# cocowy1/PPMStereo

Measured on AMD Instinct MI355X. Metric: disparity-px/s, higher is better.
Workload: dtype bf16; 1 GPU; BASELINE config 2: T=5 clip at 320x512, iters=10, hot path only (3-scale cascade from encoder outputs: corr pyramid build + lookup, QAM pick, pick-and-play memory attention, ConvGRU3D update, heads, convex upsample, test_mode=True as PPMStereo.forward_batch_test calls it: predictions[-1] is the output, so the mask head, the convex upsampling and the full-resolution resize run only where their resu; T=5, H=320, W=512, iters=10, parallelism=replicas x1

## Files before the change

### ppmstereo_amd/csrc/pwchain.hip

```cpp
#include "common.h"

namespace {

constexpr int TP = 128;
constexpr int ROWB = 64;
constexpr int ACT_PLANE = TP * ROWB;
constexpr int ACT_BUF = 4 * ACT_PLANE;
constexpr int W_BLK = 2 * 2 * 64 * 64;

__device__ __forceinline__ int swzp(int row, int chunk) { return row * 64 + ((chunk ^ ((row >> 2) & 3)) << 4); }

struct Layer {
    const void* w;
    const float* bias;
    const float* post_s;
    const float* post_t;
    int M;
    int n_valid;
    int resid;
};

struct ChainParams {
    ppms_sp in, out;
    Layer layer[3];
    int nlayers;
    int64_t P;
};

__global__ __launch_bounds__(256) void pwchain_kernel(const ChainParams* __restrict__ cp) {
    extern __shared__ __attribute__((aligned(16))) char smem[];
    const ChainParams& c = *cp;
    char* bufX = smem;
    char* bufA = smem + ACT_BUF;
    char* wsm = smem + 2 * ACT_BUF;
    const int tid = threadIdx.x, lane = tid & 63, wave = tid >> 6;
    const int r = lane & 31, h = lane >> 5;
    const int64_t p0 = (int64_t)blockIdx.x * TP;

    for (int q = tid; q < TP * 8; q += 256) {
        const int px = q >> 3, ch = q & 7;
        const int64_t pix = p0 + px;
        u32x4 vh = {0, 0, 0, 0}, vl = {0, 0, 0, 0};
        if (pix < c.P) {
            vh = gload16((const bf16_t*)c.in.hi + pix * c.in.ld + ch * 8);
            vl = gload16((const bf16_t*)c.in.lo + pix * c.in.ld + ch * 8);
        }
        const int off = (ch >> 2) * 2 * ACT_PLANE + swzp(px, ch & 3);
        *(u32x4*)(bufX + off) = vh;
        *(u32x4*)(bufX + ACT_PLANE + off) = vl;
    }
    u32x4 wreg[4];
    auto load_w = [&](int l, int mblk) __attribute__((always_inline)) {
        const Layer& Lw = c.layer[l];
        const int mbs = Lw.M / 64;
#pragma unroll
        for (int i = 0; i < 4; ++i) {
            const int q = tid + i * 256;
            const int ks = q >> 9, rem = q & 511;
            wreg[i] = gload16((const char*)Lw.w + ((int64_t)(ks * mbs + mblk) * 512 + rem) * 16);
        }
    };
    load_w(0, 0);
    const char* src = bufX;
    for (int l = 0; l < c.nlayers; ++l) {
        const Layer& L = c.layer[l];
        const bool last = (l == c.nlayers - 1);
        char* dst = (src == bufX) ? bufA : bufX;
        const int mblocks = L.M / 64;
        for (int mblk = 0; mblk < mblocks; ++mblk) {
            __syncthreads();
#pragma unroll
            for (int i = 0; i < 4; ++i) *(u32x4*)(wsm + (tid + i * 256) * 16) = wreg[i];
            if (mblk + 1 < mblocks)
                load_w(l, mblk + 1);
            else if (l + 1 < c.nlayers)
                load_w(l + 1, 0);
            __syncthreads();
            f32x16 acc[2];
            acc[0] = (f32x16){0};
            acc[1] = (f32x16){0};
#pragma unroll
            for (int ks = 0; ks < 2; ++ks) {
#pragma unroll
                for (int k16 = 0; k16 < 2; ++k16) {
                    const int boff = ks * 2 * ACT_PLANE + swzp(wave * 32 + r, 2 * k16 + h);
                    const bf16x8 bh = *(const bf16x8*)(src + boff);
                    const bf16x8 bl = *(const bf16x8*)(src + ACT_PLANE + boff);
#pragma unroll
                    for (int mb = 0; mb < 2; ++mb) {
                        const int aoff = ks * 8192 + swzp(mb * 32 + r, 2 * k16 + h);
                        const bf16x8 ah = *(const bf16x8*)(wsm + aoff);
                        const bf16x8 al = *(const bf16x8*)(wsm + 4096 + aoff);
                        acc[mb] = __builtin_amdgcn_mfma_f32_32x32x16_bf16(al, bh, acc[mb], 0, 0, 0);
                        acc[mb] = __builtin_amdgcn_mfma_f32_32x32x16_bf16(ah, bl, acc[mb], 0, 0, 0);
                        acc[mb] = __builtin_amdgcn_mfma_f32_32x32x16_bf16(ah, bh, acc[mb], 0, 0, 0);
                    }
                }
            }
            const int px = wave * 32 + r;
            const int64_t pix = p0 + px;
#pragma unroll
            for (int mb = 0; mb < 2; ++mb)
#pragma unroll
                for (int g = 0; g < 4; ++g) {
                    const int cl = mb * 32 + 8 * g + 4 * h;
                    const int cg = mblk * 64 + cl;
                    const f32x4 b4 = gld<f32x4>(L.bias + cg);
                    float y[4];
#pragma unroll
                    for (int j = 0; j < 4; ++j) y[j] = acc[mb][4 * g + j] + b4[j];
                    if (L.resid) {
                        const int xo = (cl >> 5) * 2 * ACT_PLANE + swzp(px, (cl & 31) >> 3) + (cl & 7) * 2;
                        const bf16x4 xh = *(const bf16x4*)(bufX + xo), xl = *(const bf16x4*)(bufX + ACT_PLANE + xo);
#pragma unroll
                        for (int j = 0; j < 4; ++j) y[j] += join_bf16(xh[j], xl[j]);
                    }
#pragma unroll
                    for (int j = 0; j < 4; ++j) y[j] = gelu_erf(y[j]);
                    if (L.post_s != nullptr) {
                        const f32x4 s4 = gld<f32x4>(L.post_s + cg), t4 = gld<f32x4>(L.post_t + cg);
#pragma unroll
                        for (int j = 0; j < 4; ++j) y[j] = gelu_erf(y[j] + (y[j] * s4[j] + t4[j]));
                    }
                    bf16x4 oh, ol;
#pragma unroll
                    for (int j = 0; j < 4; ++j) {
                        bf16_t hh = (bf16_t)0.0f, ll = (bf16_t)0.0f;
                        if (cg + j < L.n_valid) split_bf16(y[j], hh, ll);
                        oh[j] = hh;
                        ol[j] = ll;
                    }
                    {
                        const int xo = (cl >> 5) * 2 * ACT_PLANE + swzp(px, (cl & 31) >> 3) + (cl & 7) * 2;
                        *(bf16x4*)(dst + xo) = oh;
                        *(bf16x4*)(dst + ACT_PLANE + xo) = ol;
                    }
                }
            if (last) {
                __syncthreads();
                for (int qd = tid; qd < TP * 16; qd += 256) {
                    const int opx = qd >> 4, plane = (qd >> 3) & 1, ch = qd & 7;
                    const int64_t opix = p0 + opx;
                    const int ocg = mblk * 64 + ch * 8;
                    if (opix < c.P && ocg < L.n_valid) {
                        const u32x4 v = *(const u32x4*)(dst + (ch >> 2) * 2 * ACT_PLANE + plane * ACT_PLANE + swzp(opx, ch & 3));
                        bf16_t* op = (bf16_t*)(plane ? c.out.lo : c.out.hi) + opix * c.out.ld + ocg;
                        if (ocg + 8 <= L.n_valid) {
                            gstore16(op, v);
                        } else {
                            const bf16_t* e = (const bf16_t*)&v;
                            for (int j = 0; j < 8; ++j)
                                if (ocg + j < L.n_valid) gst<bf16_t>(op + j, e[j]);
                        }
                    }
                }
            }
        }
        src = dst;
    }
}

constexpr int TP32 = 32;
constexpr int ACT32_PLANE = TP32 * ROWB;
constexpr int ACT32_BUF = 4 * ACT32_PLANE;
constexpr int W32_MAX = 4 * W_BLK;

__global__ __launch_bounds__(256) void pwchain32_kernel(const ChainParams* __restrict__ cp) {
    extern __shared__ __attribute__((aligned(16))) char smem[];
    const ChainParams& c = *cp;
    char* bufX = smem;
    char* bufA = smem + ACT32_BUF;
    char* wsm = smem + 2 * ACT32_BUF;
    const int tid = threadIdx.x, lane = tid & 63, wave = tid >> 6;
    const int r = lane & 31, h = lane >> 5;
    const int64_t p0 = (int64_t)blockIdx.x * TP32;
    {
        const int px = tid >> 3, ch = tid & 7;
        const int64_t pix = p0 + px;
        u32x4 vh = {0, 0, 0, 0}, vl = {0, 0, 0, 0};
        if (pix < c.P) {
            vh = gload16((const bf16_t*)c.in.hi + pix * c.in.ld + ch * 8);
            vl = gload16((const bf16_t*)c.in.lo + pix * c.in.ld + ch * 8);
        }
        const int off = (ch >> 2) * 2 * ACT32_PLANE + swzp(px, ch & 3);
        *(u32x4*)(bufX + off) = vh;
        *(u32x4*)(bufX + ACT32_PLANE + off) = vl;
    }
    u32x4 wreg[16];
    auto load_w = [&](int l) __attribute__((always_inline)) {
        const Layer& Lw = c.layer[l];
        const int mbs = Lw.M / 64;
#pragma unroll
        for (int mblk = 0; mblk < 4; ++mblk)
            if (mblk < mbs) {
#pragma unroll
                for (int i = 0; i < 4; ++i) {
                    const int q = tid + i * 256;
                    const int ks = q >> 9, rem = q & 511;
                    wreg[mblk * 4 + i] = gload16((const char*)Lw.w + ((int64_t)(ks * mbs + mblk) * 512 + rem) * 16);
                }
            }
    };
    load_w(0);
    const char* src = bufX;
    for (int l = 0; l < c.nlayers; ++l) {
        const Layer& L = c.layer[l];
        const bool last = (l == c.nlayers - 1);
        char* dst = (src == bufX) ? bufA : bufX;
        const int mbs = L.M / 64, nrb = L.M / 32;
        __syncthreads();
#pragma unroll
        for (int mblk = 0; mblk < 4; ++mblk)
            if (mblk < mbs) {
#pragma unroll
                for (int i = 0; i < 4; ++i) *(u32x4*)(wsm + mblk * W_BLK + (tid + i * 256) * 16) = wreg[mblk * 4 + i];
            }
        if (l + 1 < c.nlayers) load_w(l + 1);
        __syncthreads();
        bf16x4 keep_h[2][4], keep_l[2][4];
#pragma unroll
        for (int it = 0; it < 2; ++it) {
            const int rb = wave + 4 * it;
            if (rb >= nrb) continue;
            const int mblk = rb >> 1, mb = rb & 1;
            f32x16 acc = (f32x16){0};
#pragma unroll
            for (int ks = 0; ks < 2; ++ks)
#pragma unroll
                for (int k16 = 0; k16 < 2; ++k16) {
                    const int boff = ks * 2 * ACT32_PLANE + swzp(r, 2 * k16 + h);
                    const bf16x8 bh = *(const bf16x8*)(src + boff), bl = *(const bf16x8*)(src + ACT32_PLANE + boff);
                    const int aoff = mblk * W_BLK + ks * 8192 + swzp(mb * 32 + r, 2 * k16 + h);
                    const bf16x8 ah = *(const bf16x8*)(wsm + aoff), al = *(const bf16x8*)(wsm + 4096 + aoff);
                    acc = __builtin_amdgcn_mfma_f32_32x32x16_bf16(al, bh, acc, 0, 0, 0);
                    acc = __builtin_amdgcn_mfma_f32_32x32x16_bf16(ah, bl, acc, 0, 0, 0);
                    acc = __builtin_amdgcn_mfma_f32_32x32x16_bf16(ah, bh, acc, 0, 0, 0);
                }
#pragma unroll
            for (int g = 0; g < 4; ++g) {
                const int cl = mb * 32 + 8 * g + 4 * h;
                const int cg = mblk * 64 + cl;
                const f32x4 b4 = gld<f32x4>(L.bias + cg);
                float y[4];
#pragma unroll
                for (int j = 0; j < 4; ++j) y[j] = acc[4 * g + j] + b4[j];
                const int xo = (cl >> 5) * 2 * ACT32_PLANE + swzp(r, (cl & 31) >> 3) + (cl & 7) * 2;
                if (L.resid) {
                    const bf16x4 xh = *(const bf16x4*)(bufX + xo), xl = *(const bf16x4*)(bufX + ACT32_PLANE + xo);
#pragma unroll
                    for (int j = 0; j < 4; ++j) y[j] += join_bf16(xh[j], xl[j]);
                }
#pragma unroll
                for (int j = 0; j < 4; ++j) y[j] = gelu_erf(y[j]);
                if (L.post_s != nullptr) {
                    const f32x4 s4 = gld<f32x4>(L.post_s + cg), t4 = gld<f32x4>(L.post_t + cg);
#pragma unroll
                    for (int j = 0; j < 4; ++j) y[j] = gelu_erf(y[j] + (y[j] * s4[j] + t4[j]));
                }
                bf16x4 oh, ol;
#pragma unroll
                for (int j = 0; j < 4; ++j) {
                    bf16_t hh = (bf16_t)0.0f, ll = (bf16_t)0.0f;
                    if (cg + j < L.n_valid) split_bf16(y[j], hh, ll);
                    oh[j] = hh;
                    ol[j] = ll;
                }
                if (last) {
                    keep_h[it][g] = oh;
                    keep_l[it][g] = ol;
                } else {
                    *(bf16x4*)(dst + xo) = oh;
                    *(bf16x4*)(dst + ACT32_PLANE + xo) = ol;
                }
            }
        }
        if (last) {
            __syncthreads();
            const int rowb = L.M * 2 + 16;
#pragma unroll
            for (int it = 0; it < 2; ++it) {
                const int rb = wave + 4 * it;
                if (rb >= nrb) continue;
#pragma unroll
                for (int g = 0; g < 4; ++g) {
                    const int cg = rb * 32 + 8 * g + 4 * h;
                    *(bf16x4*)(wsm + r * rowb + cg * 2) = keep_h[it][g];
                    *(bf16x4*)(wsm + TP32 * rowb + r * rowb + cg * 2) = keep_l[it][g];
                }
            }
            __syncthreads();
            const int cpr = L.M / 8;
            for (int qd = tid; qd < TP32 * 2 * cpr; qd += 256) {
                const int plane = qd / (TP32 * cpr), rem = qd - plane * TP32 * cpr;
                const int opx = rem / cpr, ch = rem - opx * cpr;
                const int64_t opix = p0 + opx;
                const int ocg = ch * 8;
                if (opix < c.P && ocg < L.n_valid) {
                    const u32x4 v = *(const u32x4*)(wsm + plane * TP32 * rowb + opx * rowb + ocg * 2);
                    bf16_t* op = (bf16_t*)(plane ? c.out.lo : c.out.hi) + opix * c.out.ld + ocg;
                    if (ocg + 8 <= L.n_valid) {
                        gstore16(op, v);
                    } else {
                        const bf16_t* e = (const bf16_t*)&v;
                        for (int j = 0; j < 8; ++j)
                            if (ocg + j < L.n_valid) gst<bf16_t>(op + j, e[j]);
                    }
                }
            }
        }
        src = dst;
    }
}

}

static int pwchain_launch(const void* dev_params, int64_t pixels, void* stream) {
    constexpr size_t lds = 2 * ACT_BUF + W_BLK;
    constexpr size_t lds32 = 2 * ACT32_BUF + W32_MAX;
    static ppms_device_once once;
    once.run([] {
        (void)hipFuncSetAttribute((const void*)pwchain_kernel, hipFuncAttributeMaxDynamicSharedMemorySize, (int)(2 * ACT_BUF + W_BLK));
        (void)hipFuncSetAttribute((const void*)pwchain32_kernel, hipFuncAttributeMaxDynamicSharedMemorySize, (int)(2 * ACT32_BUF + W32_MAX));
    });
    if (pixels <= 16384) {
        hipLaunchKernelGGL(pwchain32_kernel, dim3(ceil_div(pixels, TP32)), dim3(256), lds32, (hipStream_t)stream, (const ChainParams*)dev_params);
        return ppms_check_launch("pwchain");
    }
    hipLaunchKernelGGL(pwchain_kernel, dim3(ceil_div(pixels, TP)), dim3(256), lds, (hipStream_t)stream, (const ChainParams*)dev_params);
    return ppms_check_launch("pwchain");
}

extern "C" int ppms_pwchain(const void* dev_params, int64_t pixels, void* stream) {
    PPMS_REQUIRE(dev_params != nullptr && pixels > 0, "pwchain: bad arguments");
    return pwchain_launch(dev_params, pixels, stream);
}

extern "C" int ppms_pwchain_param_bytes(void) { return (int)sizeof(ChainParams); }
```

### ppmstereo_amd/csrc/small_ops.hip

```cpp
#include "common.h"

static thread_local char g_err[512] = "";
void ppms_set_error(const char* fmt, ...) {
    va_list ap;
    va_start(ap, fmt);
    vsnprintf(g_err, sizeof(g_err), fmt, ap);
    va_end(ap);
}
int ppms_check_launch(const char* what) {
    hipError_t e = hipGetLastError();
    if (e != hipSuccess) {
        ppms_set_error("%s: HIP launch failed: %s", what, hipGetErrorString(e));
        return PPMS_ELAUNCH;
    }
    return PPMS_OK;
}
extern "C" const char* ppms_last_error(void) { return g_err; }
extern "C" int ppms_version(void) { return PPMS_ABI_VERSION; }
extern "C" int ppms_struct_sizes(int* sp, int* epilogue, int* conv) {
    if (sp) *sp = (int)sizeof(ppms_sp);
    if (epilogue) *epilogue = (int)sizeof(ppms_epilogue);
    if (conv) *conv = (int)sizeof(ppms_conv);
    return PPMS_OK;
}
extern "C" int ppms_device_info(char* name, int name_cap, int* cu_count, int* clock_mhz) {
    int dev = 0;
    if (hipGetDevice(&dev) != hipSuccess) {
        ppms_set_error("no HIP device");
        return PPMS_ENODEV;
    }
    hipDeviceProp_t prop;
    if (hipGetDeviceProperties(&prop, dev) != hipSuccess) {
        ppms_set_error("hipGetDeviceProperties failed");
        return PPMS_ENODEV;
    }
    if (name && name_cap > 0) snprintf(name, name_cap, "%s", prop.gcnArchName);
    if (cu_count) *cu_count = prop.multiProcessorCount;
    if (clock_mhz) *clock_mhz = prop.clockRate / 1000;
    return PPMS_OK;
}

constexpr int DW_PX = 2;
template <int K>
__global__ __launch_bounds__(256) void dwconv_gelu_kernel(ppms_sp x, ppms_sp y, const float* __restrict__ w, const float* __restrict__ b,
                                                          int H, int W, int64_t rows, int groups) {
    __shared__ __attribute__((aligned(16))) float wl[K * K * 64];
    const int C = groups * 8;
    for (int i = threadIdx.x; i < K * K * C; i += 256) {
        const int c = i % C, tap = i / C;
        wl[tap * C + c] = w[c * K * K + tap];
    }
    __syncthreads();
    const int rpr = (W + DW_PX - 1) / DW_PX;
    const int64_t idx = (int64_t)blockIdx.x * 256 + threadIdx.x;
    if (idx >= rows * rpr * groups) return;
    const int c0 = (int)(idx % groups) * 8;
    const int64_t run = idx / groups;
    const int px0 = (int)(run % rpr) * DW_PX;
    const int64_t row = run / rpr;
    const int py = (int)(row % H);
    const int64_t pix0 = row * W + px0;
    const bf16_t* xh = (const bf16_t*)x.hi + c0;
    const bf16_t* xl = (const bf16_t*)x.lo + c0;
    float acc[DW_PX][8], x0[DW_PX][8];
    {
        const f32x4 b0 = *(const f32x4*)(b + c0), b1 = *(const f32x4*)(b + c0 + 4);
#pragma unroll
        for (int p = 0; p < DW_PX; ++p)
#pragma unroll
            for (int j = 0; j < 8; ++j) {
                acc[p][j] = j < 4 ? b0[j & 3] : b1[j & 3];
                x0[p][j] = 0.0f;
            }
    }
    constexpr int R = K / 2, NW = DW_PX + K - 1;
#pragma unroll
    for (int ky = 0; ky < K; ++ky) {
        const int yy = py + ky - R;
        if ((unsigned)yy >= (unsigned)H) continue;
        float win[NW][8];
#pragma unroll
        for (int i = 0; i < NW; ++i) {
            const int xx = px0 - R + i;
            bf16x8 h8 = {0, 0, 0, 0, 0, 0, 0, 0}, l8 = {0, 0, 0, 0, 0, 0, 0, 0};
            if ((unsigned)xx < (unsigned)W) {
                const int64_t q = pix0 + (int64_t)(ky - R) * W + (i - R);
                h8 = *(const bf16x8*)(xh + q * x.ld);
                l8 = *(const bf16x8*)(xl + q * x.ld);
            }
#pragma unroll
            for (int j = 0; j < 8; ++j) win[i][j] = join_bf16(h8[j], l8[j]);
        }
        if (ky == R) {
#pragma unroll
            for (int p = 0; p < DW_PX; ++p)
#pragma unroll
                for (int j = 0; j < 8; ++j) x0[p][j] = win[p + R][j];
        }
#pragma unroll
        for (int kx = 0; kx < K; ++kx) {
            const f32x4 w0 = *(const f32x4*)(wl + (ky * K + kx) * C + c0), w1 = *(const f32x4*)(wl + (ky * K + kx) * C + c0 + 4);
#pragma unroll
            for (int p = 0; p < DW_PX; ++p)
#pragma unroll
                for (int j = 0; j < 8; ++j) acc[p][j] += (j < 4 ? w0[j & 3] : w1[j & 3]) * win[p + kx][j];
        }
    }
#pragma unroll
    for (int p = 0; p < DW_PX; ++p) {
        if (px0 + p >= W) break;
        bf16x8 oh, ol;
#pragma unroll
        for (int j = 0; j < 8; ++j) {
            bf16_t hi, lo;
            split_bf16(gelu_erf(x0[p][j] + acc[p][j]), hi, lo);
            oh[j] = hi;
            ol[j] = lo;
        }
        *(bf16x8*)((bf16_t*)y.hi + (pix0 + p) * y.ld + c0) = oh;
        *(bf16x8*)((bf16_t*)y.lo + (pix0 + p) * y.ld + c0) = ol;
    }
}

extern "C" int ppms_dwconv_gelu(ppms_sp x, ppms_sp y, const float* w, const float* b, int k, int BT, int H, int W, void* stream) {
    PPMS_REQUIRE(k == 1 || k == 7, "dwconv_gelu: k=%d (only 1 and 7)", k);
    PPMS_REQUIRE(x.hi && x.lo && y.hi && y.lo && x.c == y.c && x.c > 0 && x.c <= 64 && x.c % 8 == 0 && x.ld % 8 == 0 && y.ld % 8 == 0,
                 "dwconv_gelu: views must have c <= 64 and c, ld multiples of 8");
    const int64_t rows = (int64_t)BT * H;
    const int groups = x.c / 8;
    const dim3 grid(ceil_div(rows * ((W + DW_PX - 1) / DW_PX) * groups, 256));
    if (k == 1)
        hipLaunchKernelGGL(dwconv_gelu_kernel<1>, grid, dim3(256), 0, (hipStream_t)stream, x, y, w, b, H, W, rows, groups);
    else
        hipLaunchKernelGGL(dwconv_gelu_kernel<7>, grid, dim3(256), 0, (hipStream_t)stream, x, y, w, b, H, W, rows, groups);
    return ppms_check_launch("dwconv_gelu");
}

__global__ __launch_bounds__(256) void flow_patch7_kernel(const float* __restrict__ flow, ppms_sp patch, int H, int W, int64_t P) {
    const int64_t idx = (int64_t)blockIdx.x * 256 + threadIdx.x;
    if (idx >= P * 128) return;
    const int k = (int)(idx & 127);
    const int64_t pix = idx >> 7;
    float v = 0.0f;
    if (k < 98) {
        const int tap = k >> 1, c = k & 1;
        const int ky = tap / 7, kx = tap - ky * 7;
        const int px = (int)(pix % W), py = (int)((pix / W) % H);
        const int xx = px + kx - 3, yy = py + ky - 3;
        if ((unsigned)xx < (unsigned)W && (unsigned)yy < (unsigned)H) v = flow[(pix + (int64_t)(ky - 3) * W + (kx - 3)) * 2 + c];
    }
    bf16_t hi, lo;
    split_bf16(v, hi, lo);
    ((bf16_t*)patch.hi)[pix * patch.ld + k] = hi;
    ((bf16_t*)patch.lo)[pix * patch.ld + k] = lo;
}

extern "C" int ppms_flow_patch7(const float* flow_nhwc, ppms_sp patch, int BT, int H, int W, void* stream) {
    PPMS_REQUIRE(flow_nhwc && patch.hi && patch.lo && patch.ld >= 128, "flow_patch7: bad arguments");
    const int64_t P = (int64_t)BT * H * W;
    hipLaunchKernelGGL(flow_patch7_kernel, dim3(ceil_div(P * 128, 256)), dim3(256), 0, (hipStream_t)stream, flow_nhwc, patch, H, W, P);
    return ppms_check_launch("flow_patch7");
}

__global__ __launch_bounds__(256) void unc_tail_kernel(ppms_sp x, const float* __restrict__ w, float bias, float* __restrict__ unc,
                                                       float* __restrict__ partial, int HW, int nblk) {
    __shared__ float red[16];
    const int frame = blockIdx.y, blk = blockIdx.x;
    const int sub = threadIdx.x & 15, grp = threadIdx.x >> 4;
    float wv[8];
#pragma unroll
    for (int j = 0; j < 8; ++j) wv[j] = w[sub * 8 + j];
    bf16x8 h8[16], l8[16];
#pragma unroll
    for (int it = 0; it < 16; ++it) {
        const int pin = blk * 256 + it * 16 + grp;
        const int64_t pix = (int64_t)frame * HW + (pin < HW ? pin : HW - 1);
        h8[it] = gld<bf16x8>((const bf16_t*)x.hi + pix * x.ld + sub * 8);
        l8[it] = gld<bf16x8>((const bf16_t*)x.lo + pix * x.ld + sub * 8);
    }
    float local = 0.0f;
#pragma unroll
    for (int it = 0; it < 16; ++it) {
        const int pin = blk * 256 + it * 16 + grp;
        float s = 0.0f;
#pragma unroll
        for (int j = 0; j < 8; ++j) s += wv[j] * join_bf16(h8[it][j], l8[it][j]);
        s += __shfl_xor(s, 1);
        s += __shfl_xor(s, 2);
        s += __shfl_xor(s, 4);
        s += __shfl_xor(s, 8);
        if (pin < HW && sub == 0) {
            const float u = sigmoid_f(s + bias);
            unc[(int64_t)frame * HW + pin] = u;
            local += u;
        }
    }
    if (sub == 0) red[grp] = local;
    __syncthreads();
    if (threadIdx.x == 0) {
        float t = 0.0f;
        for (int i = 0; i < 16; ++i) t += red[i];
        partial[frame * nblk + blk] = t;
    }
}

extern "C" int ppms_unc_tail(ppms_sp x, const float* w, float bias, float* unc, float* partial, int BT, int HW, void* stream) {
    PPMS_REQUIRE(x.hi && x.lo && x.c == 128 && x.ld % 8 == 0, "unc_tail: expects a 128-channel SP view");
    const int nblk = ceil_div(HW, 256);
    hipLaunchKernelGGL(unc_tail_kernel, dim3(nblk, BT), dim3(256), 0, (hipStream_t)stream, x, w, bias, unc, partial, HW, nblk);
    return ppms_check_launch("unc_tail");
}

enum { CV_F32 = 0, CV_SP = 1 };
template <int DST_KIND>
__global__ __launch_bounds__(256) void nchw_to_cl_kernel(const float* __restrict__ src, float* __restrict__ dst_f32, int dst_ld,
                                                         ppms_sp dst_sp, int C, int HW) {
    __shared__ float tile[32][33];
    const int frame = blockIdx.z;
    const int c0 = blockIdx.y * 32, p0 = blockIdx.x * 32;
    const int tx = threadIdx.x & 31, ty = threadIdx.x >> 5;
    for (int i = ty; i < 32; i += 8) {
        const int c = c0 + i, p = p0 + tx;
        tile[i][tx] = (c < C && p < HW) ? src[((int64_t)frame * C + c) * HW + p] : 0.0f;
    }
    __syncthreads();
    for (int i = ty; i < 32; i += 8) {
        const int p = p0 + i, c = c0 + tx;
        if (p < HW && c < C) {
            const float v = tile[tx][i];
            const int64_t pix = (int64_t)frame * HW + p;
            if (DST_KIND == CV_F32) {
                dst_f32[pix * dst_ld + c] = v;
            } else {
                bf16_t hi, lo;
                split_bf16(v, hi, lo);
                ((bf16_t*)dst_sp.hi)[pix * dst_sp.ld + c] = hi;
                ((bf16_t*)dst_sp.lo)[pix * dst_sp.ld + c] = lo;
            }
        }
    }
}
template <int SRC_KIND>
__global__ __launch_bounds__(256) void cl_to_nchw_kernel(const float* __restrict__ src_f32, int src_ld, ppms_sp src_sp,
                                                         float* __restrict__ dst, int C, int HW) {
    __shared__ float tile[32][33];
    const int frame = blockIdx.z;
    const int c0 = blockIdx.y * 32, p0 = blockIdx.x * 32;
    const int tx = threadIdx.x & 31, ty = threadIdx.x >> 5;
    for (int i = ty; i < 32; i += 8) {
        const int p = p0 + i, c = c0 + tx;
        float v = 0.0f;
        if (p < HW && c < C) {
            const int64_t pix = (int64_t)frame * HW + p;
            if (SRC_KIND == CV_F32)
                v = src_f32[pix * src_ld + c];
            else
                v = join_bf16(((const bf16_t*)src_sp.hi)[pix * src_sp.ld + c], ((const bf16_t*)src_sp.lo)[pix * src_sp.ld + c]);
        }
        tile[i][tx] = v;
    }
    __syncthreads();
    for (int i = ty; i < 32; i += 8) {
        const int c = c0 + i, p = p0 + tx;
        if (c < C && p < HW) dst[((int64_t)frame * C + c) * HW + p] = tile[tx][i];
    }
}

extern "C" int ppms_nchw_to_sp(const float* src, ppms_sp dst, int BT, int C, int HW, void* stream) {
    PPMS_REQUIRE(src && dst.hi && dst.lo && dst.ld >= C, "nchw_to_sp: bad arguments");
    hipLaunchKernelGGL(nchw_to_cl_kernel<CV_SP>, dim3(ceil_div(HW, 32), ceil_div(C, 32), BT), dim3(256), 0, (hipStream_t)stream, src,
                       (float*)nullptr, 0, dst, C, HW);
    return ppms_check_launch("nchw_to_sp");
}
extern "C" int ppms_nchw_to_nhwc(const float* src, float* dst, int dst_ld, int BT, int C, int HW, void* stream) {
    PPMS_REQUIRE(src && dst && dst_ld >= C, "nchw_to_nhwc: bad arguments");
    ppms_sp none = {nullptr, nullptr, 0, 0};
    hipLaunchKernelGGL(nchw_to_cl_kernel<CV_F32>, dim3(ceil_div(HW, 32), ceil_div(C, 32), BT), dim3(256), 0, (hipStream_t)stream, src, dst,
                       dst_ld, none, C, HW);
    return ppms_check_launch("nchw_to_nhwc");
}
extern "C" int ppms_sp_to_nchw(ppms_sp src, float* dst, int BT, int C, int HW, void* stream) {
    PPMS_REQUIRE(dst && src.hi && src.lo && src.ld >= C, "sp_to_nchw: bad arguments");
    hipLaunchKernelGGL(cl_to_nchw_kernel<CV_SP>, dim3(ceil_div(HW, 32), ceil_div(C, 32), BT), dim3(256), 0, (hipStream_t)stream,
                       (const float*)nullptr, 0, src, dst, C, HW);
    return ppms_check_launch("sp_to_nchw");
}
extern "C" int ppms_nhwc_to_nchw(const float* src, int src_ld, float* dst, int BT, int C, int HW, void* stream) {
    PPMS_REQUIRE(src && dst && src_ld >= C, "nhwc_to_nchw: bad arguments");
    ppms_sp none = {nullptr, nullptr, 0, 0};
    hipLaunchKernelGGL(cl_to_nchw_kernel<CV_F32>, dim3(ceil_div(HW, 32), ceil_div(C, 32), BT), dim3(256), 0, (hipStream_t)stream, src,
                       src_ld, none, dst, C, HW);
    return ppms_check_launch("nhwc_to_nchw");
}

__global__ __launch_bounds__(256) void f32_to_sp_kernel(const float* __restrict__ src, int src_ld, ppms_sp dst, int64_t n) {
    const int64_t idx = (int64_t)blockIdx.x * 256 + threadIdx.x;
    if (idx >= n) return;
    const int c = (int)(idx % dst.c);
    const int64_t pix = idx / dst.c;
    bf16_t hi, lo;
    split_bf16(src[pix * src_ld + c], hi, lo);
    ((bf16_t*)dst.hi)[pix * dst.ld + c] = hi;
    ((bf16_t*)dst.lo)[pix * dst.ld + c] = lo;
}
__global__ __launch_bounds__(256) void sp_to_f32_kernel(ppms_sp src, float* __restrict__ dst, int dst_ld, int64_t n) {
    const int64_t idx = (int64_t)blockIdx.x * 256 + threadIdx.x;
    if (idx >= n) return;
    const int c = (int)(idx % src.c);
    const int64_t pix = idx / src.c;
    dst[pix * dst_ld + c] = join_bf16(((const bf16_t*)src.hi)[pix * src.ld + c], ((const bf16_t*)src.lo)[pix * src.ld + c]);
}
extern "C" int ppms_f32_to_sp(const float* src, int src_ld, ppms_sp dst, int64_t pixels, void* stream) {
    PPMS_REQUIRE(src && dst.hi && dst.lo && dst.c > 0, "f32_to_sp: bad arguments");
    const int64_t n = pixels * dst.c;
    hipLaunchKernelGGL(f32_to_sp_kernel, dim3(ceil_div(n, 256)), dim3(256), 0, (hipStream_t)stream, src, src_ld, dst, n);
    return ppms_check_launch("f32_to_sp");
}
extern "C" int ppms_sp_to_f32(ppms_sp src, float* dst, int dst_ld, int64_t pixels, void* stream) {
    PPMS_REQUIRE(dst && src.hi && src.lo && src.c > 0, "sp_to_f32: bad arguments");
    const int64_t n = pixels * src.c;
    hipLaunchKernelGGL(sp_to_f32_kernel, dim3(ceil_div(n, 256)), dim3(256), 0, (hipStream_t)stream, src, dst, dst_ld, n);
    return ppms_check_launch("sp_to_f32");
}

__global__ __launch_bounds__(256) void tap_gather_sum_kernel(const float* __restrict__ y, int y_ld, const float* __restrict__ bias,
                                                             float* __restrict__ out, int out_ld, float* __restrict__ accum, int accum_ld, int cout,
                                                             int kt, int kh, int kw, int T, int H, int W, int t_halo, int64_t total) {
    const int64_t idx = (int64_t)blockIdx.x * 256 + threadIdx.x;
    if (idx >= total) return;
    const int c = (int)(idx % cout);
    const int64_t pix = idx / cout;
    const int x = (int)(pix % W), yy = (int)((pix / W) % H), t = (int)(pix / ((int64_t)W * H));
    float acc = bias ? bias[c] : 0.0f;
    int tap = 0;
    for (int kz = 0; kz < kt; ++kz)
        for (int ky = 0; ky < kh; ++ky)
            for (int kx = 0; kx < kw; ++kx, ++tap) {
                const int tt = t + kz - kt / 2, y2 = yy + ky - kh / 2, x2 = x + kx - kw / 2;
                if ((unsigned)(tt + t_halo) < (unsigned)(T + 2 * t_halo) && (unsigned)y2 < (unsigned)H && (unsigned)x2 < (unsigned)W)
                    acc += y[(((int64_t)tt * H + y2) * W + x2) * y_ld + tap * cout + c];
            }
    out[pix * out_ld + c] = acc;
    if (accum != nullptr) accum[pix * accum_ld + c] += acc;
}
__global__ __launch_bounds__(256) void tap_gather_sum333_kernel(const float* __restrict__ y, int y_ld, const float* __restrict__ bias,
                                                                float* __restrict__ out, int out_ld, float* __restrict__ accum, int accum_ld, int cout,
                                                                int T, int H, int W, int t_halo, int64_t total) {
    const int64_t idx = (int64_t)blockIdx.x * 256 + threadIdx.x;
    if (idx >= total) return;
    const int c = (int)(idx % cout);
    const int64_t pix = idx / cout;
    const int x = (int)(pix % W), yy = (int)((pix / W) % H), t = (int)(pix / ((int64_t)W * H));
    float v[27];
#pragma unroll
    for (int tap = 0; tap < 27; ++tap) {
        const int kz = tap / 9, ky = (tap / 3) % 3, kx = tap % 3;
        const int tt = t + kz - 1, y2 = yy + ky - 1, x2 = x + kx - 1;
        const bool ok = (unsigned)(tt + t_halo) < (unsigned)(T + 2 * t_halo) && (unsigned)y2 < (unsigned)H && (unsigned)x2 < (unsigned)W;
        v[tap] = ok ? y[(((int64_t)tt * H + y2) * W + x2) * y_ld + tap * cout + c] : 0.0f;
    }
    float acc = bias ? bias[c] : 0.0f;
#pragma unroll
    for (int tap = 0; tap < 27; ++tap) {
        const int kz = tap / 9, ky = (tap / 3) % 3, kx = tap % 3;
        const int tt = t + kz - 1, y2 = yy + ky - 1, x2 = x + kx - 1;
        const bool ok = (unsigned)(tt + t_halo) < (unsigned)(T + 2 * t_halo) && (unsigned)y2 < (unsigned)H && (unsigned)x2 < (unsigned)W;
        if (ok) acc += v[tap];
    }
    out[pix * out_ld + c] = acc;
    if (accum != nullptr) accum[pix * accum_ld + c] += acc;
}
extern "C" int ppms_tap_gather_sum(const float* y, int y_ld, const float* bias, float* out, int out_ld, float* accum, int accum_ld, int cout, int kt,
                                   int kh, int kw, int T, int H, int W, int t_halo, void* stream) {
    PPMS_REQUIRE(y && out && cout > 0 && kt * kh * kw * cout <= y_ld && out_ld >= cout && t_halo >= 0, "tap_gather_sum: bad arguments");
    PPMS_REQUIRE(accum == nullptr || accum_ld >= cout, "tap_gather_sum: accum_ld=%d < cout=%d", accum_ld, cout);
    const int64_t total = (int64_t)T * H * W * cout;
    if (kt == 3 && kh == 3 && kw == 3)
        hipLaunchKernelGGL(tap_gather_sum333_kernel, dim3(ceil_div(total, 256)), dim3(256), 0, (hipStream_t)stream, y, y_ld, bias, out, out_ld, accum,
                           accum_ld, cout, T, H, W, t_halo, total);
    else
        hipLaunchKernelGGL(tap_gather_sum_kernel, dim3(ceil_div(total, 256)), dim3(256), 0, (hipStream_t)stream, y, y_ld, bias, out, out_ld, accum, accum_ld,
                           cout, kt, kh, kw, T, H, W, t_halo, total);
    return ppms_check_launch("tap_gather_sum");
}

__global__ __launch_bounds__(256) void flow_add_kernel(float* __restrict__ flow, const float* __restrict__ dflow, int dflow_ld, int64_t P) {
    const int64_t idx = (int64_t)blockIdx.x * 256 + threadIdx.x;
    if (idx >= P * 2) return;
    flow[idx] += dflow[(idx >> 1) * dflow_ld + (idx & 1)];
}
extern "C" int ppms_flow_add(float* flow_nhwc, const float* dflow, int dflow_ld, int64_t pixels, void* stream) {
    PPMS_REQUIRE(flow_nhwc && dflow && dflow_ld >= 2, "flow_add: bad arguments");
    hipLaunchKernelGGL(flow_add_kernel, dim3(ceil_div(pixels * 2, 256)), dim3(256), 0, (hipStream_t)stream, flow_nhwc, dflow, dflow_ld, pixels);
    return ppms_check_launch("flow_add");
}

__global__ __launch_bounds__(256) void convex_upsample_kernel(const float* __restrict__ flow, const float* __restrict__ mask, int mask_ld,
                                                              float* __restrict__ out, int H, int W, int64_t P) {
    const int64_t idx = (int64_t)blockIdx.x * 256 + threadIdx.x;
    if (idx >= P * 16) return;
    const int sub = (int)(idx & 15);
    const int64_t pix = idx >> 4;
    const int x = (int)(pix % W), y = (int)((pix / W) % H);
    const int64_t frame = pix / ((int64_t)H * W);
    const float* m = mask + pix * mask_ld + sub;
    float mv[9], mx = -INFINITY;
#pragma unroll
    for (int k = 0; k < 9; ++k) {
        mv[k] = m[16 * k];
        mx = fmaxf(mx, mv[k]);
    }
    float den = 0.0f;
#pragma unroll
    for (int k = 0; k < 9; ++k) {
        mv[k] = expf(mv[k] - mx);
        den += mv[k];
    }
    float o0 = 0.0f, o1 = 0.0f;
#pragma unroll
    for (int k = 0; k < 9; ++k) {
        const int yy = y + k / 3 - 1, xx = x + k % 3 - 1;
        if ((unsigned)yy < (unsigned)H && (unsigned)xx < (unsigned)W) {
            const int64_t q = pix + (int64_t)(k / 3 - 1) * W + (k % 3 - 1);
            const float wgt = mv[k] / den;
            o0 += wgt * (4.0f * flow[q * 2]);
            o1 += wgt * (4.0f * flow[q * 2 + 1]);
        }
    }
    const int i = sub >> 2, j = sub & 3;
    const int64_t OW = 4 * (int64_t)W, OHW = 16 * (int64_t)H * W;
    const int64_t o = (frame * 2) * OHW + (int64_t)(4 * y + i) * OW + 4 * x + j;
    out[o] = o0;
    out[o + OHW] = o1;
}
extern "C" int ppms_convex_upsample(const float* flow_nhwc, const float* mask, int mask_ld, float* out, int BT, int H, int W, void* stream) {
    PPMS_REQUIRE(flow_nhwc && mask && out && mask_ld >= 144, "convex_upsample: bad arguments");
    const int64_t P = (int64_t)BT * H * W;
// ... 524 lines not shown
```

Before: 23.09 million disparity-px/s.

## Tile depthwise 7x7 conv through LDS and skip padded channel blocks in pwchain

Replaces the per-pixel 7x7 depthwise GELU kernel with a tiled kernel that stages a haloed input tile (converted to fp32) and transposed weights in shared memory. Tile size is picked by CU count. This removes redundant global reads of neighbouring pixels. The pointwise chain kernels now hoist bias and post-scale loads ahead of the MFMA loop, skip MFMA and epilogue work for 32-channel blocks beyond n_valid, and request two blocks per CU via launch bounds. The costs are larger LDS use per block and possible register pressure from the occupancy hint.

```diff
diff --git a/ppmstereo_amd/csrc/pwchain.hip b/ppmstereo_amd/csrc/pwchain.hip
--- a/ppmstereo_amd/csrc/pwchain.hip
+++ b/ppmstereo_amd/csrc/pwchain.hip
@@ -27,7 +27,7 @@
     int64_t P;
 };
 
-__global__ __launch_bounds__(256) void pwchain_kernel(const ChainParams* __restrict__ cp) {
+__global__ __launch_bounds__(256, 2) void pwchain_kernel(const ChainParams* __restrict__ cp) {
     extern __shared__ __attribute__((aligned(16))) char smem[];
     const ChainParams& c = *cp;
     char* bufX = smem;
@@ -76,6 +76,21 @@
             else if (l + 1 < c.nlayers)
                 load_w(l + 1, 0);
             __syncthreads();
+            const int nv = L.n_valid, cb = mblk * 64;
+            f32x4 b4[2][4], s4[2][4], t4[2][4];
+#pragma unroll
+            for (int mb = 0; mb < 2; ++mb)
+#pragma unroll
+                for (int g = 0; g < 4; ++g) {
+                    const int cg = cb + mb * 32 + 8 * g + 4 * h;
+                    if (cb + mb * 32 + 8 * g < nv) {
+                        b4[mb][g] = gld<f32x4>(L.bias + cg);
+                        if (L.post_s != nullptr) {
+                            s4[mb][g] = gld<f32x4>(L.post_s + cg);
+                            t4[mb][g] = gld<f32x4>(L.post_t + cg);
+                        }
+                    }
+                }
             f32x16 acc[2];
             acc[0] = (f32x16){0};
             acc[1] = (f32x16){0};
@@ -88,6 +103,7 @@
                     const bf16x8 bl = *(const bf16x8*)(src + ACT_PLANE + boff);
 #pragma unroll
                     for (int mb = 0; mb < 2; ++mb) {
+                        if (cb + mb * 32 >= nv) continue;
                         const int aoff = ks * 8192 + swzp(mb * 32 + r, 2 * k16 + h);
                         const bf16x8 ah = *(const bf16x8*)(wsm + aoff);
                         const bf16x8 al = *(const bf16x8*)(wsm + 4096 + aoff);
@@ -105,30 +121,31 @@
                 for (int g = 0; g < 4; ++g) {
                     const int cl = mb * 32 + 8 * g + 4 * h;
                     const int cg = mblk * 64 + cl;
-                    const f32x4 b4 = gld<f32x4>(L.bias + cg);
-                    float y[4];
-#pragma unroll
-                    for (int j = 0; j < 4; ++j) y[j] = acc[mb][4 * g + j] + b4[j];
-                    if (L.resid) {
-                        const int xo = (cl >> 5) * 2 * ACT_PLANE + swzp(px, (cl & 31) >> 3) + (cl & 7) * 2;
-                        const bf16x4 xh = *(const bf16x4*)(bufX + xo), xl = *(const bf16x4*)(bufX + ACT_PLANE + xo);
-#pragma unroll
-                        for (int j = 0; j < 4; ++j) y[j] += join_bf16(xh[j], xl[j]);
-                    }
-#pragma unroll
-                    for (int j = 0; j < 4; ++j) y[j] = gelu_erf(y[j]);
-                    if (L.post_s != nullptr) {
-                        const f32x4 s4 = gld<f32x4>(L.post_s + cg), t4 = gld<f32x4>(L.post_t + cg);
-#pragma unroll
-                        for (int j = 0; j < 4; ++j) y[j] = gelu_erf(y[j] + (y[j] * s4[j] + t4[j]));
-                    }
-                    bf16x4 oh, ol;
-#pragma unroll
-                    for (int j = 0; j < 4; ++j) {
-                        bf16_t hh = (bf16_t)0.0f, ll = (bf16_t)0.0f;
-                        if (cg + j < L.n_valid) split_bf16(y[j], hh, ll);
-                        oh[j] = hh;
-                        ol[j] = ll;
+                    const bf16_t z = (bf16_t)0.0f;
+                    bf16x4 oh = {z, z, z, z}, ol = {z, z, z, z};
+                    if (cb + mb * 32 + 8 * g < nv) {
+                        float y[4];
+#pragma unroll
+                        for (int j = 0; j < 4; ++j) y[j] = acc[mb][4 * g + j] + b4[mb][g][j];
+                        if (L.resid) {
+                            const int xo = (cl >> 5) * 2 * ACT_PLANE + swzp(px, (cl & 31) >> 3) + (cl & 7) * 2;
+                            const bf16x4 xh = *(const bf16x4*)(bufX + xo), xl = *(const bf16x4*)(bufX + ACT_PLANE + xo);
+#pragma unroll
+                            for (int j = 0; j < 4; ++j) y[j] += join_bf16(xh[j], xl[j]);
+                        }
+#pragma unroll
+                        for (int j = 0; j < 4; ++j) y[j] = gelu_erf(y[j]);
+                        if (L.post_s != nullptr) {
+#pragma unroll
+                            for (int j = 0; j < 4; ++j) y[j] = gelu_erf(y[j] + (y[j] * s4[mb][g][j] + t4[mb][g][j]));
+                        }
+#pragma unroll
+                        for (int j = 0; j < 4; ++j) {
+                            bf16_t hh = z, ll = z;
+                            if (cg + j < nv) split_bf16(y[j], hh, ll);
+                            oh[j] = hh;
+                            ol[j] = ll;
+                        }
                     }
                     {
                         const int xo = (cl >> 5) * 2 * ACT_PLANE + swzp(px, (cl & 31) >> 3) + (cl & 7) * 2;
@@ -165,7 +182,7 @@
 constexpr int ACT32_BUF = 4 * ACT32_PLANE;
 constexpr int W32_MAX = 4 * W_BLK;
 
-__global__ __launch_bounds__(256) void pwchain32_kernel(const ChainParams* __restrict__ cp) {
+__global__ __launch_bounds__(256, 2) void pwchain32_kernel(const ChainParams* __restrict__ cp) {
     extern __shared__ __attribute__((aligned(16))) char smem[];
     const ChainParams& c = *cp;
     char* bufX = smem;
@@ -223,47 +240,63 @@
             const int rb = wave + 4 * it;
             if (rb >= nrb) continue;
             const int mblk = rb >> 1, mb = rb & 1;
+            const int nv = L.n_valid, rb0 = rb * 32;
+            f32x4 b4[4], s4[4], t4[4];
+#pragma unroll
+            for (int g = 0; g < 4; ++g) {
+                const int cg = rb0 + 8 * g + 4 * h;
+                if (rb0 + 8 * g < nv) {
+                    b4[g] = gld<f32x4>(L.bias + cg);
+                    if (L.post_s != nullptr) {
+                        s4[g] = gld<f32x4>(L.post_s + cg);
+                        t4[g] = gld<f32x4>(L.post_t + cg);
+                    }
+                }
+            }
             f32x16 acc = (f32x16){0};
-#pragma unroll
-            for (int ks = 0; ks < 2; ++ks)
-#pragma unroll
-                for (int k16 = 0; k16 < 2; ++k16) {
-                    const int boff = ks * 2 * ACT32_PLANE + swzp(r, 2 * k16 + h);
-                    const bf16x8 bh = *(const bf16x8*)(src + boff), bl = *(const bf16x8*)(src + ACT32_PLANE + boff);
-                    const int aoff = mblk * W_BLK + ks * 8192 + swzp(mb * 32 + r, 2 * k16 + h);
-                    const bf16x8 ah = *(const bf16x8*)(wsm + aoff), al = *(const bf16x8*)(wsm + 4096 + aoff);
-                    acc = __builtin_amdgcn_mfma_f32_32x32x16_bf16(al, bh, acc, 0, 0, 0);
-                    acc = __builtin_amdgcn_mfma_f32_32x32x16_bf16(ah, bl, acc, 0, 0, 0);
-                    acc = __builtin_amdgcn_mfma_f32_32x32x16_bf16(ah, bh, acc, 0, 0, 0);
-                }
+            if (rb0 < nv) {
+#pragma unroll
+                for (int ks = 0; ks < 2; ++ks)
+#pragma unroll
+                    for (int k16 = 0; k16 < 2; ++k16) {
+                        const int boff = ks * 2 * ACT32_PLANE + swzp(r, 2 * k16 + h);
+                        const bf16x8 bh = *(const bf16x8*)(src + boff), bl = *(const bf16x8*)(src + ACT32_PLANE + boff);
+                        const int aoff = mblk * W_BLK + ks * 8192 + swzp(mb * 32 + r, 2 * k16 + h);
+                        const bf16x8 ah = *(const bf16x8*)(wsm + aoff), al = *(const bf16x8*)(wsm + 4096 + aoff);
+                        acc = __builtin_amdgcn_mfma_f32_32x32x16_bf16(al, bh, acc, 0, 0, 0);
+                        acc = __builtin_amdgcn_mfma_f32_32x32x16_bf16(ah, bl, acc, 0, 0, 0);
+                        acc = __builtin_amdgcn_mfma_f32_32x32x16_bf16(ah, bh, acc, 0, 0, 0);
+                    }
+            }
 #pragma unroll
             for (int g = 0; g < 4; ++g) {
                 const int cl = mb * 32 + 8 * g + 4 * h;
                 const int cg = mblk * 64 + cl;
-                const f32x4 b4 = gld<f32x4>(L.bias + cg);
-                float y[4];
-#pragma unroll
-                for (int j = 0; j < 4; ++j) y[j] = acc[4 * g + j] + b4[j];
                 const int xo = (cl >> 5) * 2 * ACT32_PLANE + swzp(r, (cl & 31) >> 3) + (cl & 7) * 2;
-                if (L.resid) {
-                    const bf16x4 xh = *(const bf16x4*)(bufX + xo), xl = *(const bf16x4*)(bufX + ACT32_PLANE + xo);
-#pragma unroll
-                    for (int j = 0; j < 4; ++j) y[j] += join_bf16(xh[j], xl[j]);
-                }
-#pragma unroll
-                for (int j = 0; j < 4; ++j) y[j] = gelu_erf(y[j]);
-                if (L.post_s != nullptr) {
-                    const f32x4 s4 = gld<f32x4>(L.post_s + cg), t4 = gld<f32x4>(L.post_t + cg);
-#pragma unroll
-                    for (int j = 0; j < 4; ++j) y[j] = gelu_erf(y[j] + (y[j] * s4[j] + t4[j]));
-                }
-                bf16x4 oh, ol;
-#pragma unroll
-                for (int j = 0; j < 4; ++j) {
-                    bf16_t hh = (bf16_t)0.0f, ll = (bf16_t)0.0f;
-                    if (cg + j < L.n_valid) split_bf16(y[j], hh, ll);
-                    oh[j] = hh;
-                    ol[j] = ll;
+                const bf16_t z = (bf16_t)0.0f;
+                bf16x4 oh = {z, z, z, z}, ol = {z, z, z, z};
+                if (rb0 + 8 * g < nv) {
+                    float y[4];
+#pragma unroll
+                    for (int j = 0; j < 4; ++j) y[j] = acc[4 * g + j] + b4[g][j];
+                    if (L.resid) {
+                        const bf16x4 xh = *(const bf16x4*)(bufX + xo), xl = *(const bf16x4*)(bufX + ACT32_PLANE + xo);
+#pragma unroll
+                        for (int j = 0; j < 4; ++j) y[j] += join_bf16(xh[j], xl[j]);
+                    }
+#pragma unroll
+                    for (int j = 0; j < 4; ++j) y[j] = gelu_erf(y[j]);
+                    if (L.post_s != nullptr) {
+#pragma unroll
+                        for (int j = 0; j < 4; ++j) y[j] = gelu_erf(y[j] + (y[j] * s4[g][j] + t4[g][j]));
+                    }
+#pragma unroll
+                    for (int j = 0; j < 4; ++j) {
+                        bf16_t hh = z, ll = z;
+                        if (cg + j < nv) split_bf16(y[j], hh, ll);
+                        oh[j] = hh;
+                        ol[j] = ll;
+                    }
                 }
                 if (last) {
                     keep_h[it][g] = oh;
diff --git a/ppmstereo_amd/csrc/small_ops.hip b/ppmstereo_amd/csrc/small_ops.hip
--- a/ppmstereo_amd/csrc/small_ops.hip
+++ b/ppmstereo_amd/csrc/small_ops.hip
@@ -122,17 +122,146 @@
     }
 }
 
+constexpr int DW7_R = 3;
+template <int TW, int TH, int NT>
+__global__ __launch_bounds__(NT) void dwconv7_tile_kernel(ppms_sp x, ppms_sp y, const float* __restrict__ w, const float* __restrict__ b,
+                                                          int H, int W, int groups, int tiles_x, int tiles_y) {
+    extern __shared__ __attribute__((aligned(16))) float dw_smem[];
+    constexpr int HW_ = TW + 2 * DW7_R, HH_ = TH + 2 * DW7_R, NPOS = HW_ * HH_, NPX = TW * TH;
+    const int C = groups * 8, CP = C + 4;
+    float* xs = dw_smem;
+    float* wl = dw_smem + NPOS * CP;
+    float* bl = wl + 49 * C;
+    const int tid = threadIdx.x;
+    const int tile = blockIdx.x;
+    const int tx0 = (tile % tiles_x) * TW;
+    const int ty0 = ((tile / tiles_x) % tiles_y) * TH;
+    const int64_t frame = tile / (tiles_x * tiles_y);
+    const int64_t row0 = frame * H;
+    constexpr int WIT = (49 * 64 + NT - 1) / NT;
+    constexpr int XIT = (NPOS * 8 + NT - 1) / NT;
+    const int nw = 49 * C;
+    float wv[WIT];
+#pragma unroll
+    for (int k = 0; k < WIT; ++k) {
+        const int i = tid + k * NT;
+        wv[k] = w[i < nw ? i : nw - 1];
+    }
+    const float bv = b[tid < C ? tid : C - 1];
+    bf16x8 h8[XIT], l8[XIT];
+    {
+        const bf16_t* xh = (const bf16_t*)x.hi;
+        const bf16_t* xl = (const bf16_t*)x.lo;
+#pragma unroll
+        for (int k = 0; k < XIT; ++k) {
+            const int q = tid + k * NT;
+            const int pos = q >> 3, ch = q & 7;
+            const int hy = pos / HW_, hx = pos - hy * HW_;
+            const int gy = ty0 + hy - DW7_R, gx = tx0 + hx - DW7_R;
+            const bool in = pos < NPOS && ch < groups && (unsigned)gy < (unsigned)H && (unsigned)gx < (unsigned)W;
+            const int64_t o = in ? ((row0 + gy) * W + gx) * x.ld + ch * 8 : 0;
+            h8[k] = *(const bf16x8*)(xh + o);
+            l8[k] = *(const bf16x8*)(xl + o);
+        }
+    }
+#pragma unroll
+    for (int k = 0; k < WIT; ++k) {
+        const int i = tid + k * NT;
+        const int c = i / 49, tap = i - c * 49;
+        if (i < nw) wl[tap * C + c] = wv[k];
+    }
+    if (tid < C) bl[tid] = bv;
+#pragma unroll
+    for (int k = 0; k < XIT; ++k) {
+        const int q = tid + k * NT;
+        const int pos = q >> 3, ch = q & 7;
+        const int hy = pos / HW_, hx = pos - hy * HW_;
+        const int gy = ty0 + hy - DW7_R, gx = tx0 + hx - DW7_R;
+        const bool in = (unsigned)gy < (unsigned)H && (unsigned)gx < (unsigned)W;
+        if (pos < NPOS && ch < groups) {
+            f32x4 v0, v1;
+#pragma unroll
+            for (int j = 0; j < 4; ++j) {
+                v0[j] = in ? join_bf16(h8[k][j], l8[k][j]) : 0.0f;
+                v1[j] = in ? join_bf16(h8[k][4 + j], l8[k][4 + j]) : 0.0f;
+            }
+            *(f32x4*)(xs + pos * CP + ch * 8) = v0;
+            *(f32x4*)(xs + pos * CP + ch * 8 + 4) = v1;
+        }
+    }
+    __syncthreads();
+    for (int item = tid; item < NPX * groups; item += NT) {
+        const int g = item / NPX, p = item - g * NPX;
+        const int ly = p / TW, lx = p - ly * TW;
+        const int gy = ty0 + ly, gx = tx0 + lx;
+        if (gy >= H || gx >= W) continue;
+        const int c0 = g * 8;
+        float acc[8];
+        {
+            const f32x4 b0 = *(const f32x4*)(bl + c0), b1 = *(const f32x4*)(bl + c0 + 4);
+#pragma unroll
+            for (int j = 0; j < 8; ++j) acc[j] = j < 4 ? b0[j & 3] : b1[j & 3];
+        }
+        const float* xp = xs + (ly * HW_ + lx) * CP + c0;
+#pragma unroll
+        for (int ky = 0; ky < 7; ++ky) {
+            if ((unsigned)(gy + ky - DW7_R) >= (unsigned)H) continue;
+#pragma unroll
+            for (int kx = 0; kx < 7; ++kx) {
+                const float* xq = xp + (ky * HW_ + kx) * CP;
+                const f32x4 x0 = *(const f32x4*)xq, x1 = *(const f32x4*)(xq + 4);
+                const f32x4 w0 = *(const f32x4*)(wl + (ky * 7 + kx) * C + c0), w1 = *(const f32x4*)(wl + (ky * 7 + kx) * C + c0 + 4);
+#pragma unroll
+                for (int j = 0; j < 8; ++j) acc[j] += (j < 4 ? w0[j & 3] : w1[j & 3]) * (j < 4 ? x0[j & 3] : x1[j & 3]);
+            }
+        }
+        const float* xc = xp + (DW7_R * HW_ + DW7_R) * CP;
+        const f32x4 c0v = *(const f32x4*)xc, c1v = *(const f32x4*)(xc + 4);
+        bf16x8 oh, ol;
+#pragma unroll
+        for (int j = 0; j < 8; ++j) {
+            bf16_t hi, lo;
+            split_bf16(gelu_erf((j < 4 ? c0v[j & 3] : c1v[j & 3]) + acc[j]), hi, lo);
+            oh[j] = hi;
+            ol[j] = lo;
+        }
+        const int64_t pix = (row0 + gy) * W + gx;
+        *(bf16x8*)((bf16_t*)y.hi + pix * y.ld + c0) = oh;
+        *(bf16x8*)((bf16_t*)y.lo + pix * y.ld + c0) = ol;
+    }
+}
+
+template <int TW, int TH, int NT>
+static int dwconv7_tile_launch(ppms_sp x, ppms_sp y, const float* w, const float* b, int BT, int H, int W, void* stream) {
+    constexpr int NPOS = (TW + 2 * DW7_R) * (TH + 2 * DW7_R);
+    constexpr int LDS_MAX = (NPOS * 68 + 50 * 64) * 4;
+    static ppms_device_once once;
+    once.run([] { (void)hipFuncSetAttribute((const void*)dwconv7_tile_kernel<TW, TH, NT>, hipFuncAttributeMaxDynamicSharedMemorySize, LDS_MAX); });
+    const int tiles_x = ceil_div(W, TW), tiles_y = ceil_div(H, TH);
+    const int64_t tiles = (int64_t)tiles_x * tiles_y * BT;
+    PPMS_REQUIRE(tiles <= 0x7fffffff, "dwconv_gelu: %lld tiles exceed one grid", (long long)tiles);
+    const size_t lds = (size_t)(NPOS * (x.c + 4) + 50 * x.c) * 4;
+    hipLaunchKernelGGL((dwconv7_tile_kernel<TW, TH, NT>), dim3((unsigned)tiles), dim3(NT), lds, (hipStream_t)stream, x, y, w, b, H, W, x.c / 8, tiles_x,
+                       tiles_y);
+    return ppms_check_launch("dwconv_gelu");
+}
+
 extern "C" int ppms_dwconv_gelu(ppms_sp x, ppms_sp y, const float* w, const float* b, int k, int BT, int H, int W, void* stream) {
     PPMS_REQUIRE(k == 1 || k == 7, "dwconv_gelu: k=%d (only 1 and 7)", k);
     PPMS_REQUIRE(x.hi && x.lo && y.hi && y.lo && x.c == y.c && x.c > 0 && x.c <= 64 && x.c % 8 == 0 && x.ld % 8 == 0 && y.ld % 8 == 0,
                  "dwconv_gelu: views must have c <= 64 and c, ld multiples of 8");
+    PPMS_REQUIRE(BT > 0 && H > 0 && W > 0, "dwconv_gelu: BT=%d, H=%d, W=%d must be positive", BT, H, W);
+    if (k == 7) {
+        const int64_t ncu = ppms_num_cus();
+        auto tiles = [&](int tw, int th) { return (int64_t)ceil_div(W, tw) * ceil_div(H, th) * BT; };
+        if (tiles(16, 8) >= ncu) return dwconv7_tile_launch<16, 8, 640>(x, y, w, b, BT, H, W, stream);
+        if (tiles(8, 4) >= ncu) return dwconv7_tile_launch<8, 4, 192>(x, y, w, b, BT, H, W, stream);
+        return dwconv7_tile_launch<4, 3, 64>(x, y, w, b, BT, H, W, stream);
+    }
     const int64_t rows = (int64_t)BT * H;
     const int groups = x.c / 8;
     const dim3 grid(ceil_div(rows * ((W + DW_PX - 1) / DW_PX) * groups, 256));
-    if (k == 1)
-        hipLaunchKernelGGL(dwconv_gelu_kernel<1>, grid, dim3(256), 0, (hipStream_t)stream, x, y, w, b, H, W, rows, groups);
-    else
-        hipLaunchKernelGGL(dwconv_gelu_kernel<7>, grid, dim3(256), 0, (hipStream_t)stream, x, y, w, b, H, W, rows, groups);
+    hipLaunchKernelGGL(dwconv_gelu_kernel<1>, grid, dim3(256), 0, (hipStream_t)stream, x, y, w, b, H, W, rows, groups);
     return ppms_check_launch("dwconv_gelu");
 }
 
```

Result: no change. 23.22 million disparity-px/s, median of 6 (+0.6%).
